# Wangshihu12/colmap-pcd

Hardware: AMD Instinct MI355X
Metric: NN queries/sec + BA-iter ms, 10M-pt cloud / 1M 3D feats (higher is better)
Workload: dtype f32 (NN distances) / f64 (association, BA); 1 GPU; M: 10000000-pt 'planes' cloud / 1000000 queries + BA scene 1000 cams / 1000000 pts / 4721253 obs / 900000 lidar terms (OPENCV), the same total at every N; cloud_points=10000000, queries=1000000, queries_this_rank=1000000, parallelism=single GPU

## Files before the change

### colmap-pcd_amd/csrc/ba.hip

```cpp
#include <algorithm>
#include <chrono>
#include <cmath>
#include <limits>
#include <memory>
#include <numeric>

#include "ba_cam_jac.h"
#include "ba_math.h"
#include "common.h"

namespace pcd {

struct BaDev {
  const int* cam_model; const int* cam_off; const double* cam_params;
  const double* poses; const int* image_cam; const uint8_t* image_const_pose; const uint8_t* image_const_tvec;
  const double* points; const uint8_t* point_const;
  const int* obs_image; const int* obs_point; const double* obs_xy;
  const int* lidar_point; const double* lidar_abcd; const double* lidar_w;
  const int* pt_order;
  const uint32_t* slice_start;
  const int* sell_img;
  const double* sell_xy;
  const uint32_t* pt_lidar_start; const uint32_t* pt_lidar_list;
  const uint32_t* img_obs_start;
  const int* img_pt;
  const uint32_t* img_obs;
  const uint32_t* seg_img;
  const uint32_t* seg_begin;
  const uint32_t* img_seg_start;
  const uint8_t* cam_refine;
  const uint32_t* cam_img_start;
  const uint32_t* cam_img_list;
  int C;
  int cam_k;
  const double* img_xy;
  int I, P, nslices; uint64_t O, L;
  int loss_type; double loss_scale;
};

template <int MODEL>
__device__ __forceinline__ void eval_block(const BaDev& d, int im, const double X[3], double ox, double oy,
                                           ReprojBlock& b, double q[4]) {
  const double* pose = d.poses + 7 * (size_t)im;
  double t[3];
#pragma unroll
  for (int k = 0; k < 4; ++k) q[k] = pose[k];
#pragma unroll
  for (int k = 0; k < 3; ++k) t[k] = pose[4 + k];
  const int cm = d.image_cam[im];
  const int model = MODEL >= 0 ? MODEL : d.cam_model[cm];
  reproj_eval(model, d.cam_params + d.cam_off[cm], q, t, X, ox, oy, b);
}

template <int N>
__device__ __forceinline__ void wave_store_rows(double* __restrict__ out, uint64_t row0, int cnt, const double (&v)[N],
                                                double* __restrict__ lds) {
  static_assert(N % 2 == 0, "rows are moved in 16-byte units");
  const int lane = threadIdx.x & 63;
#pragma unroll
  for (int k = 0; k < N; ++k) lds[lane * N + k] = v[k];
  __builtin_amdgcn_fence(__ATOMIC_RELEASE, "workgroup");
  __builtin_amdgcn_wave_barrier();
  __builtin_amdgcn_fence(__ATOMIC_ACQUIRE, "workgroup");
  const double2* src = reinterpret_cast<const double2*>(lds);
  double2* dst = reinterpret_cast<double2*>(out + row0 * N);
  const int units = cnt * (N / 2);
#pragma unroll
  for (int j = 0; j < N / 2; ++j) {
    const int u = j * 64 + lane;
    if (u < units) dst[u] = src[u];
  }
  __builtin_amdgcn_fence(__ATOMIC_RELEASE, "workgroup");
  __builtin_amdgcn_wave_barrier();
}

template <int MODEL, bool BLOCKS>
__global__ __launch_bounds__(256) void k_ba_points(BaDev d, double* __restrict__ Hpt, double* __restrict__ gpt,
                                                   double* __restrict__ cost_partial) {
  __shared__ double s_half[2][64][9];
  const int sl = threadIdx.x >> 7, half = (threadIdx.x >> 6) & 1, lane = threadIdx.x & 63;
  const int slice = blockIdx.x * 2 + sl;
  const int t = slice * 64 + lane;
  double cost = 0.0;
  double H[6] = {0, 0, 0, 0, 0, 0}, g[3] = {0, 0, 0};
  int p = -1;
  bool cpt = true;
  double X[3] = {0, 0, 0};
  if (slice < d.nslices) {
    p = d.pt_order[t];
    const uint32_t s0 = d.slice_start[slice], s1 = d.slice_start[slice + 1];
    if (p >= 0) {
      X[0] = d.points[3 * (size_t)p]; X[1] = d.points[3 * (size_t)p + 1]; X[2] = d.points[3 * (size_t)p + 2];
      cpt = d.point_const && d.point_const[p];
    }
    for (uint32_t s = s0 + lane + 64u * half; s < s1; s += 128) {
      const int im = d.sell_img[s];
      if (im < 0) continue;
      ReprojBlock b;
      double q[4];
      eval_block<MODEL>(d, im, X, d.sell_xy[2 * (size_t)s], d.sell_xy[2 * (size_t)s + 1], b, q);
      double rho0, rho1;
      loss_eval(d.loss_type, d.loss_scale, b.r[0] * b.r[0] + b.r[1] * b.r[1], rho0, rho1);
      cost += 0.5 * rho0;
      if (BLOCKS && !cpt) {
        const double sr = sqrt(rho1);
        double J[6];
#pragma unroll
        for (int r = 0; r < 2; ++r)
#pragma unroll
          for (int k = 0; k < 3; ++k)
            J[3 * r + k] = sr * (b.M[3 * r] * b.D[k] + b.M[3 * r + 1] * b.D[3 + k] + b.M[3 * r + 2] * b.D[6 + k]);
        const double r0 = sr * b.r[0], r1 = sr * b.r[1];
        H[0] += J[0] * J[0] + J[3] * J[3]; H[1] += J[0] * J[1] + J[3] * J[4]; H[2] += J[0] * J[2] + J[3] * J[5];
        H[3] += J[1] * J[1] + J[4] * J[4]; H[4] += J[1] * J[2] + J[4] * J[5]; H[5] += J[2] * J[2] + J[5] * J[5];
        g[0] += J[0] * r0 + J[3] * r1; g[1] += J[1] * r0 + J[4] * r1; g[2] += J[2] * r0 + J[5] * r1;
      }
    }
  }
  if (BLOCKS && half == 1) {
#pragma unroll
    for (int k = 0; k < 6; ++k) s_half[sl][lane][k] = H[k];
#pragma unroll
    for (int k = 0; k < 3; ++k) s_half[sl][lane][6 + k] = g[k];
  }
  __syncthreads();
  if (half == 0 && slice < d.nslices) {
    if (BLOCKS) {
#pragma unroll
      for (int k = 0; k < 6; ++k) H[k] += s_half[sl][lane][k];
#pragma unroll
      for (int k = 0; k < 3; ++k) g[k] += s_half[sl][lane][6 + k];
    }
    if (p >= 0) {
      for (uint32_t e = d.pt_lidar_start[p]; e < d.pt_lidar_start[p + 1]; ++e) {
        const uint32_t l = d.pt_lidar_list[e];
        const double abcd[4] = {d.lidar_abcd[4 * (size_t)l], d.lidar_abcd[4 * (size_t)l + 1],
                                d.lidar_abcd[4 * (size_t)l + 2], d.lidar_abcd[4 * (size_t)l + 3]};
        double r, J[3];
        lidar_eval(X, abcd, d.lidar_w[l], 0, r, J);
        double rho0, rho1;
        loss_eval(d.loss_type, d.loss_scale, r * r, rho0, rho1);
        cost += 0.5 * rho0;
        if (BLOCKS && !cpt) {
          const double sr = sqrt(rho1);
          const double rc = sr * r;
          J[0] *= sr; J[1] *= sr; J[2] *= sr;
          H[0] += J[0] * J[0]; H[1] += J[0] * J[1]; H[2] += J[0] * J[2];
          H[3] += J[1] * J[1]; H[4] += J[1] * J[2]; H[5] += J[2] * J[2];
          g[0] += J[0] * rc; g[1] += J[1] * rc; g[2] += J[2] * rc;
        }
      }
      if (BLOCKS && Hpt) {
        double* h = Hpt + 9 * (size_t)p;
        h[0] = H[0]; h[1] = H[1]; h[2] = H[2]; h[3] = H[1]; h[4] = H[3]; h[5] = H[4]; h[6] = H[2]; h[7] = H[4]; h[8] = H[5];
      }
      if (BLOCKS && gpt) { gpt[3 * (size_t)p] = g[0]; gpt[3 * (size_t)p + 1] = g[1]; gpt[3 * (size_t)p + 2] = g[2]; }
    }
  }
  __syncthreads();
  __shared__ double s_c[256];
  s_c[threadIdx.x] = cost;
  __syncthreads();
  for (int off = 128; off > 0; off >>= 1) {
    if ((int)threadIdx.x < off) s_c[threadIdx.x] += s_c[threadIdx.x + off];
    __syncthreads();
  }
  if (threadIdx.x == 0) cost_partial[blockIdx.x] = s_c[0];
}

template <int MODEL>
__global__ __launch_bounds__(256) void k_ba_cost(BaDev d, double* __restrict__ cost_partial) {
  double cost = 0.0;
  for (uint64_t i = blockIdx.x * (uint64_t)256 + threadIdx.x; i < d.O + d.L; i += (uint64_t)gridDim.x * 256) {
    if (i < d.O) {
      const int im = d.obs_image[i], pt = d.obs_point[i];
      const double X[3] = {d.points[3 * (size_t)pt], d.points[3 * (size_t)pt + 1], d.points[3 * (size_t)pt + 2]};
      ReprojBlock b;
      double q[4];
      eval_block<MODEL>(d, im, X, d.obs_xy[2 * i], d.obs_xy[2 * i + 1], b, q);
      double rho0, rho1;
      loss_eval(d.loss_type, d.loss_scale, b.r[0] * b.r[0] + b.r[1] * b.r[1], rho0, rho1);
      cost += 0.5 * rho0;
    } else {
      const uint64_t l = i - d.O;
      const int pt = d.lidar_point[l];
      const double X[3] = {d.points[3 * (size_t)pt], d.points[3 * (size_t)pt + 1], d.points[3 * (size_t)pt + 2]};
      const double abcd[4] = {d.lidar_abcd[4 * l], d.lidar_abcd[4 * l + 1], d.lidar_abcd[4 * l + 2], d.lidar_abcd[4 * l + 3]};
      double r, J[3];
      lidar_eval(X, abcd, d.lidar_w[l], 0, r, J);
      double rho0, rho1;
      loss_eval(d.loss_type, d.loss_scale, r * r, rho0, rho1);
      cost += 0.5 * rho0;
    }
  }
  __shared__ double s_c[256];
  s_c[threadIdx.x] = cost;
  __syncthreads();
  for (int off = 128; off > 0; off >>= 1) {
    if ((int)threadIdx.x < off) s_c[threadIdx.x] += s_c[threadIdx.x + off];
    __syncthreads();
  }
  if (threadIdx.x == 0) cost_partial[blockIdx.x] = s_c[0];
}
constexpr unsigned kCostBlocks = 1u << 20;

__global__ __launch_bounds__(256) void k_sum_partials(const double* __restrict__ partial, int n, double* __restrict__ out) {
  __shared__ double s_c[256];
  double a0 = 0.0, a1 = 0.0, a2 = 0.0, a3 = 0.0;
  int i = threadIdx.x;
  for (; i + 768 < n; i += 1024) { a0 += partial[i]; a1 += partial[i + 256]; a2 += partial[i + 512]; a3 += partial[i + 768]; }
  for (; i < n; i += 256) a0 += partial[i];
  s_c[threadIdx.x] = (a0 + a1) + (a2 + a3);
  __syncthreads();
  for (int off = 128; off > 0; off >>= 1) {
    if ((int)threadIdx.x < off) s_c[threadIdx.x] += s_c[threadIdx.x + off];
    __syncthreads();
  }
  if (threadIdx.x == 0) out[0] = s_c[0];
}

constexpr uint32_t kImgSeg = 1024;
template <int MODEL, bool WANT_W>
__global__ __launch_bounds__(256) void k_ba_images(BaDev d, double* __restrict__ partial, double* __restrict__ W_o) {
  __shared__ __attribute__((aligned(16))) double s_w[WANT_W ? 4 : 1][WANT_W ? 64 * 18 : 2];
  const int im = (int)d.seg_img[blockIdx.x];
  const int lane = threadIdx.x & 63;
  const int wave = __builtin_amdgcn_readfirstlane((int)(threadIdx.x >> 6));
  const bool cpose = d.image_const_pose && d.image_const_pose[im];
  double acc[27];
#pragma unroll
  for (int k = 0; k < 27; ++k) acc[k] = 0.0;
  const unsigned tmask = d.image_const_tvec ? d.image_const_tvec[im] : 0u;
  const uint32_t e_beg = d.seg_begin[blockIdx.x];
  const uint32_t e_end = min(d.seg_begin[blockIdx.x + 1], d.img_obs_start[im + 1]);
  if (!cpose || WANT_W) {
    for (uint32_t e0 = e_beg; e0 < e_end; e0 += 256) {
      const uint32_t e = e0 + threadIdx.x;
      const bool active = e < e_end;
      double w[18];
#pragma unroll
      for (int k = 0; k < 18; ++k) w[k] = 0.0;
      if (active && !cpose) {
        const int pt = d.img_pt[e];
        const double X[3] = {d.points[3 * (size_t)pt], d.points[3 * (size_t)pt + 1], d.points[3 * (size_t)pt + 2]};
        ReprojBlock b;
        double q[4];
        eval_block<MODEL>(d, im, X, d.img_xy[2 * (size_t)e], d.img_xy[2 * (size_t)e + 1], b, q);
        double rho0, rho1;
        loss_eval(d.loss_type, d.loss_scale, b.r[0] * b.r[0] + b.r[1] * b.r[1], rho0, rho1);
        const double sr = sqrt(rho1);
        double Jq[8], Jt[6], JX[6], Jqt[6];
        reproj_jacobians(b, Jq, Jt, JX);
        quat_tangent(q, Jq, Jqt);
        double J[12];
#pragma unroll
        for (int r = 0; r < 2; ++r)
#pragma unroll
          for (int k = 0; k < 3; ++k) {
            J[6 * r + k] = sr * Jqt[3 * r + k];
            J[6 * r + 3 + k] = ((tmask >> k) & 1u) ? 0.0 : sr * Jt[3 * r + k];
          }
        const double r0 = sr * b.r[0], r1 = sr * b.r[1];
        int idx = 0;
#pragma unroll
        for (int a = 0; a < 6; ++a)
#pragma unroll
          for (int c = a; c < 6; ++c) acc[idx++] += J[a] * J[c] + J[6 + a] * J[6 + c];
#pragma unroll
        for (int a = 0; a < 6; ++a) acc[21 + a] += J[a] * r0 + J[6 + a] * r1;
        if (WANT_W && !(d.point_const && d.point_const[pt])) {
#pragma unroll
          for (int a = 0; a < 6; ++a)
#pragma unroll
            for (int c = 0; c < 3; ++c) w[3 * a + c] = J[a] * (sr * JX[c]) + J[6 + a] * (sr * JX[3 + c]);
        }
      }
      if (WANT_W) {
        const uint32_t o = active ? d.img_obs[e] : 0u;
        const uint32_t o_first = (uint32_t)__builtin_amdgcn_readfirstlane((int)o);
        const int cnt = (int)min(64u, e_end > e0 + wave * 64u ? e_end - (e0 + wave * 64u) : 0u);
        const bool contiguous = __all(!active || o == o_first + (uint32_t)lane);
        if (contiguous) {
          wave_store_rows<18>(W_o, o_first, cnt, w, s_w[wave]);
        } else if (active) {
          double* dst = W_o + 18 * (size_t)o;
#pragma unroll
          for (int k = 0; k < 18; ++k) dst[k] = w[k];
        }
      }
    }
  }
  __shared__ double s_a[4][27];
#pragma unroll
  for (int k = 0; k < 27; ++k) {
    double v = acc[k];
#pragma unroll
    for (int off = 32; off > 0; off >>= 1) v += __shfl_xor(v, off);
    if (lane == 0) s_a[wave][k] = v;
  }
  __syncthreads();
  if (threadIdx.x < 27)
    partial[27 * (size_t)blockIdx.x + threadIdx.x] =
        (s_a[0][threadIdx.x] + s_a[1][threadIdx.x]) + (s_a[2][threadIdx.x] + s_a[3][threadIdx.x]);
}

__global__ __launch_bounds__(64) void k_ba_images_reduce(BaDev d, const double* __restrict__ partial,
                                                         double* __restrict__ Himg, double* __restrict__ gimg) {
  const int im = blockIdx.x * 2 + (threadIdx.x >> 5), k = threadIdx.x & 31;
  if (im >= d.I || k >= 27) return;
  double v = 0.0;
  for (uint32_t sgm = d.img_seg_start[im]; sgm < d.img_seg_start[im + 1]; ++sgm) v += partial[27 * (size_t)sgm + k];
  if (k >= 21) {
    if (gimg) gimg[6 * (size_t)im + (k - 21)] = v;
  } else if (Himg) {
    int a = 0, kk = k;
    while (kk >= 6 - a) { kk -= 6 - a; ++a; }
    const int c = a + kk;
    Himg[36 * (size_t)im + 6 * a + c] = v;
    Himg[36 * (size_t)im + 6 * c + a] = v;
  }
}

__host__ __device__ constexpr int cam_ne(int K) { return K * (K + 1) / 2 + 6 * K + K; }
__host__ __device__ constexpr int cam_ent_l(int K, int e) {
  const int ncc = K * (K + 1) / 2;
  if (e < ncc) { int a = 0; while (e >= K - a) { e -= K - a; ++a; } return a; }
  e -= ncc;
  if (e < 6 * K) return e / 6;
  return e - 6 * K;
}
__host__ __device__ constexpr int cam_ent_r(int K, int e) {
  const int ncc = K * (K + 1) / 2;
  if (e < ncc) { int a = 0; while (e >= K - a) { e -= K - a; ++a; } return a + e; }
  e -= ncc;
  if (e < 6 * K) return K + e % 6;
  return K + 6;
}

template <int MODEL, int CH>
__device__ __forceinline__ void cam_accumulate(const BaDev& d, int im, double* __restrict__ partial) {
  constexpr int K = MODEL >= 0 ? cam_num_params(MODEL >= 0 ? MODEL : 0) : PCD_CAM_JAC_STRIDE;
  constexpr int NE = cam_ne(K), PER = (NE + 3) / 4, E0 = CH * PER, E1 = E0 + PER < NE ? E0 + PER : NE;
  constexpr int NA = K + 7;
  const int lane = threadIdx.x & 63;
  const bool cpose = d.image_const_pose && d.image_const_pose[im];
  const unsigned tmask = d.image_const_tvec ? d.image_const_tvec[im] : 0u;
  const int cm = d.image_cam[im];
  const double* cam = d.cam_params + d.cam_off[cm];
  const uint8_t* refine = d.cam_refine ? d.cam_refine + d.cam_off[cm] : nullptr;
  const int model = MODEL >= 0 ? MODEL : d.cam_model[cm];
  double acc[PER > 0 ? PER : 1];
#pragma unroll
  for (int t = 0; t < PER; ++t) acc[t] = 0.0;
  for (uint32_t e = d.img_obs_start[im] + lane; e < d.img_obs_start[im + 1]; e += 64) {
    const int pt = d.img_pt[e];
    const double X[3] = {d.points[3 * (size_t)pt], d.points[3 * (size_t)pt + 1], d.points[3 * (size_t)pt + 2]};
    ReprojBlock b;
    double q[4];
    eval_block<MODEL>(d, im, X, d.img_xy[2 * (size_t)e], d.img_xy[2 * (size_t)e + 1], b, q);
    double rho0, rho1;
    loss_eval(d.loss_type, d.loss_scale, b.r[0] * b.r[0] + b.r[1] * b.r[1], rho0, rho1);
    const double sr = sqrt(rho1);
    double A[2][NA];
    {
      const double* pose = d.poses + 7 * (size_t)im;
      const double w = pose[0], a = pose[1], bq = pose[2], c = pose[3];
      const double cx = bq * X[2] - c * X[1], cy = c * X[0] - a * X[2], cz = a * X[1] - bq * X[0];
      const double ux = 2.0 * cx, uy = 2.0 * cy, uz = 2.0 * cz;
      const double Px = X[0] + w * ux + (bq * uz - c * uy) + pose[4];
      const double Py = X[1] + w * uy + (c * ux - a * uz) + pose[5];
      const double Pz = X[2] + w * uz + (a * uy - bq * ux) + pose[6];
      const double iz = 1.0 / Pz;
      double Jc[2 * K];
#pragma unroll
      for (int k = 0; k < 2 * K; ++k) Jc[k] = 0.0;
      if (MODEL >= 0) cam_param_jacobian<(MODEL >= 0 ? MODEL : 0)>(cam, Px * iz, Py * iz, Jc, K);
      else cam_param_jacobian_any(model, cam, Px * iz, Py * iz, Jc, K);
      const int kn = MODEL >= 0 ? K : cam_num_params(model);
#pragma unroll
      for (int k = 0; k < K; ++k) {
        const bool var = refine && k < kn && refine[k < kn ? k : 0];
        A[0][k] = var ? sr * Jc[k] : 0.0;
        A[1][k] = var ? sr * Jc[K + k] : 0.0;
      }
    }
    double Jq[8], Jt[6], JX[6], Jqt[6];
    reproj_jacobians(b, Jq, Jt, JX);
    quat_tangent(q, Jq, Jqt);
#pragma unroll
    for (int r = 0; r < 2; ++r) {
#pragma unroll
      for (int k = 0; k < 3; ++k) {
        A[r][K + k] = cpose ? 0.0 : sr * Jqt[3 * r + k];
        A[r][K + 3 + k] = (cpose || ((tmask >> k) & 1u)) ? 0.0 : sr * Jt[3 * r + k];
      }
      A[r][K + 6] = sr * b.r[r];
    }
#pragma unroll
    for (int t = 0; t < PER; ++t) {
      if (E0 + t < E1) {
        const int l = cam_ent_l(K, E0 + t), r = cam_ent_r(K, E0 + t);
        acc[t] += A[0][l] * A[0][r] + A[1][l] * A[1][r];
      }
    }
  }
#pragma unroll
  for (int t = 0; t < PER; ++t) {
    if (E0 + t < E1) {
      double v = acc[t];
#pragma unroll
      for (int off = 32; off > 0; off >>= 1) v += __shfl_xor(v, off);
      if (lane == 0) partial[(size_t)im * cam_ne(PCD_CAM_JAC_STRIDE) + E0 + t] = v;
    }
  }
}

template <int MODEL>
__global__ __launch_bounds__(256) void k_ba_cameras(BaDev d, double* __restrict__ partial) {
  const int im = blockIdx.x;
  switch (threadIdx.x >> 6) {
    case 0: cam_accumulate<MODEL, 0>(d, im, partial); break;
    case 1: cam_accumulate<MODEL, 1>(d, im, partial); break;
    case 2: cam_accumulate<MODEL, 2>(d, im, partial); break;
    default: cam_accumulate<MODEL, 3>(d, im, partial); break;
  }
}

__global__ __launch_bounds__(256) void k_ba_cameras_reduce(BaDev d, const double* __restrict__ partial,
                                                           double* __restrict__ Hcam, double* __restrict__ gcam,
                                                           double* __restrict__ Ecam) {
  constexpr int S = PCD_CAM_JAC_STRIDE, NEMAX = cam_ne(S);
  const int c = blockIdx.x;
  const int model = d.cam_model[c];
  const int K = d.cam_k;
  (void)model;
  const int ncc = K * (K + 1) / 2, NE = ncc + 7 * K;
  for (int e = threadIdx.x; e < S * S + S; e += 256) {
    if (e < S * S) { if (Hcam) Hcam[(size_t)c * S * S + e] = 0.0; }
    else if (gcam) gcam[(size_t)c * S + (e - S * S)] = 0.0;
  }
  __syncthreads();
  for (int e = threadIdx.x; e < NE; e += 256) {
    if (e >= ncc && e < ncc + 6 * K) continue;
    double v = 0.0;
    for (uint32_t j = d.cam_img_start[c]; j < d.cam_img_start[c + 1]; ++j)
      v += partial[(size_t)d.cam_img_list[j] * NEMAX + e];
    if (e < ncc) {
      int a = 0, k = e;
      while (k >= K - a) { k -= K - a; ++a; }
      const int b = a + k;
      if (Hcam) { Hcam[(size_t)c * S * S + a * S + b] = v; Hcam[(size_t)c * S * S + b * S + a] = v; }
    } else if (gcam) {
      gcam[(size_t)c * S + (e - ncc - 6 * K)] = v;
    }
  }
  if (Ecam) {
    for (uint32_t j = d.cam_img_start[c]; j < d.cam_img_start[c + 1]; ++j) {
      const uint32_t im = d.cam_img_list[j];
      for (int e = threadIdx.x; e < S * 6; e += 256) {
        const int a = e / 6;
        Ecam[(size_t)im * S * 6 + e] = a < K ? partial[(size_t)im * NEMAX + ncc + e] : 0.0;
      }
    }
  }
}

template <int MODEL>
__global__ __launch_bounds__(256) void k_ba_cam_w(BaDev d, double* __restrict__ Wc_o) {
  constexpr int S = PCD_CAM_JAC_STRIDE;
  __shared__ __attribute__((aligned(16))) double s_rows[4][64 * 3 * S];
  const int wave = threadIdx.x >> 6;
  const uint64_t o = blockIdx.x * (uint64_t)256 + threadIdx.x;
  const uint64_t o_wave = blockIdx.x * (uint64_t)256 + wave * 64;
  if (o_wave >= d.O) return;
  const int cnt = (int)min((uint64_t)64, d.O - o_wave);
  double Wc[3 * S];
#pragma unroll
  for (int k = 0; k < 3 * S; ++k) Wc[k] = 0.0;
  if (o < d.O) {
    const int im = d.obs_image[o], pt = d.obs_point[o];
    const bool cpt = d.point_const && d.point_const[pt];
    const int cm = d.image_cam[im];
    const uint8_t* refine = d.cam_refine ? d.cam_refine + d.cam_off[cm] : nullptr;
    if (!cpt && refine) {
      const double X[3] = {d.points[3 * (size_t)pt], d.points[3 * (size_t)pt + 1], d.points[3 * (size_t)pt + 2]};
      ReprojBlock b;
      double q[4];
      eval_block<MODEL>(d, im, X, d.obs_xy[2 * o], d.obs_xy[2 * o + 1], b, q);
      double rho0, rho1;
      loss_eval(d.loss_type, d.loss_scale, b.r[0] * b.r[0] + b.r[1] * b.r[1], rho0, rho1);
      double Jq[8], Jt[6], JX[6];
      reproj_jacobians(b, Jq, Jt, JX);
      const double* pose = d.poses + 7 * (size_t)im;
      const double w = pose[0], a = pose[1], bq = pose[2], c = pose[3];
      const double cx = bq * X[2] - c * X[1], cy = c * X[0] - a * X[2], cz = a * X[1] - bq * X[0];
      const double ux = 2.0 * cx, uy = 2.0 * cy, uz = 2.0 * cz;
      const double Px = X[0] + w * ux + (bq * uz - c * uy) + pose[4];
      const double Py = X[1] + w * uy + (c * ux - a * uz) + pose[5];
      const double Pz = X[2] + w * uz + (a * uy - bq * ux) + pose[6];
      const double iz = 1.0 / Pz;
      const int model = MODEL >= 0 ? MODEL : d.cam_model[cm];
      double Jc[2 * S];
#pragma unroll
      for (int k = 0; k < 2 * S; ++k) Jc[k] = 0.0;
      if (MODEL >= 0) cam_param_jacobian<(MODEL >= 0 ? MODEL : 0)>(d.cam_params + d.cam_off[cm], Px * iz, Py * iz, Jc, S);
      else cam_param_jacobian_any(model, d.cam_params + d.cam_off[cm], Px * iz, Py * iz, Jc, S);
      const int kn = cam_num_params(model);
#pragma unroll
      for (int k = 0; k < S; ++k) {
        const bool var = k < kn && refine[k < kn ? k : 0];
#pragma unroll
        for (int j = 0; j < 3; ++j)
          Wc[3 * k + j] = var ? rho1 * (Jc[k] * JX[j] + Jc[S + k] * JX[3 + j]) : 0.0;
      }
    }
  }
  wave_store_rows<3 * S>(Wc_o, o_wave, cnt, Wc, s_rows[wave]);
}

template <int MODEL>
__global__ __launch_bounds__(256) void k_ba_raw(BaDev d, double* __restrict__ residuals, double* __restrict__ Jq_o,
                                                double* __restrict__ Jt_o, double* __restrict__ JX_o,
                                                double* __restrict__ W_o) {
  __shared__ __attribute__((aligned(16))) double s_rows[4][64 * 18];
  const int wave = threadIdx.x >> 6;
  const uint64_t o = blockIdx.x * (uint64_t)256 + threadIdx.x;
  const uint64_t o_wave = blockIdx.x * (uint64_t)256 + wave * 64;
  if (o_wave >= d.O) return;
  const int cnt = (int)min((uint64_t)64, d.O - o_wave);
  const bool active = o < d.O;
  double res[2] = {0, 0}, Jq[8], Jt[6], JX[6], Wb[18];
#pragma unroll
  for (int k = 0; k < 8; ++k) Jq[k] = 0.0;
#pragma unroll
  for (int k = 0; k < 6; ++k) { Jt[k] = 0.0; JX[k] = 0.0; }
#pragma unroll
  for (int k = 0; k < 18; ++k) Wb[k] = 0.0;
  if (active) {
    const int im = d.obs_image[o], pt = d.obs_point[o];
    const double X[3] = {d.points[3 * (size_t)pt], d.points[3 * (size_t)pt + 1], d.points[3 * (size_t)pt + 2]};
    ReprojBlock b;
    double q[4];
    eval_block<MODEL>(d, im, X, d.obs_xy[2 * o], d.obs_xy[2 * o + 1], b, q);
    reproj_jacobians(b, Jq, Jt, JX);
    const bool cpose = d.image_const_pose && d.image_const_pose[im];
    res[0] = b.r[0]; res[1] = b.r[1];
    if (W_o) {
      double rho0, rho1;
      loss_eval(d.loss_type, d.loss_scale, b.r[0] * b.r[0] + b.r[1] * b.r[1], rho0, rho1);
      const double sr = sqrt(rho1);
      const unsigned tmask = d.image_const_tvec ? d.image_const_tvec[im] : 0u;
      const bool cpt = d.point_const && d.point_const[pt];
      double Jqt[6], J[12], Jx[6];
      quat_tangent(q, Jq, Jqt);
#pragma unroll
      for (int r = 0; r < 2; ++r)
#pragma unroll
        for (int k = 0; k < 3; ++k) {
          J[6 * r + k] = cpose ? 0.0 : sr * Jqt[3 * r + k];
          J[6 * r + 3 + k] = (cpose || ((tmask >> k) & 1u)) ? 0.0 : sr * Jt[3 * r + k];
          Jx[3 * r + k] = cpt ? 0.0 : sr * JX[3 * r + k];
        }
#pragma unroll
      for (int a = 0; a < 6; ++a)
#pragma unroll
        for (int c = 0; c < 3; ++c) Wb[3 * a + c] = J[a] * Jx[c] + J[6 + a] * Jx[3 + c];
    }
    if (cpose) {
#pragma unroll
      for (int k = 0; k < 8; ++k) Jq[k] = 0.0;
#pragma unroll
      for (int k = 0; k < 6; ++k) Jt[k] = 0.0;
    }
  }
  if (residuals) wave_store_rows<2>(residuals, o_wave, cnt, res, s_rows[wave]);
  if (Jq_o) wave_store_rows<8>(Jq_o, o_wave, cnt, Jq, s_rows[wave]);
  if (Jt_o) wave_store_rows<6>(Jt_o, o_wave, cnt, Jt, s_rows[wave]);
  if (JX_o) wave_store_rows<6>(JX_o, o_wave, cnt, JX, s_rows[wave]);
  if (W_o) wave_store_rows<18>(W_o, o_wave, cnt, Wb, s_rows[wave]);
}

template <int MODEL>
__global__ __launch_bounds__(256) void k_ba_cam_jac(BaDev d, double* __restrict__ Jc_o) {
  const uint64_t o = blockIdx.x * (uint64_t)256 + threadIdx.x;
  if (o >= d.O) return;
  const int im = d.obs_image[o], pt = d.obs_point[o];
  const double* pose = d.poses + 7 * (size_t)im;
  const double* Xp = d.points + 3 * (size_t)pt;
  const double X[3] = {Xp[0], Xp[1], Xp[2]};
  const double w = pose[0], a = pose[1], bq = pose[2], c = pose[3];
  const double cx = bq * X[2] - c * X[1], cy = c * X[0] - a * X[2], cz = a * X[1] - bq * X[0];
  const double ux = 2.0 * cx, uy = 2.0 * cy, uz = 2.0 * cz;
  const double Px = X[0] + w * ux + (bq * uz - c * uy) + pose[4];
  const double Py = X[1] + w * uy + (c * ux - a * uz) + pose[5];
  const double Pz = X[2] + w * uz + (a * uy - bq * ux) + pose[6];
  const double iz = 1.0 / Pz;
  const int cm = d.image_cam[im];
  double J[2 * PCD_CAM_JAC_STRIDE];
#pragma unroll
  for (int k = 0; k < 2 * PCD_CAM_JAC_STRIDE; ++k) J[k] = 0.0;
  if (MODEL >= 0) cam_param_jacobian<(MODEL >= 0 ? MODEL : 0)>(d.cam_params + d.cam_off[cm], Px * iz, Py * iz, J, PCD_CAM_JAC_STRIDE);
  else cam_param_jacobian_any(d.cam_model[cm], d.cam_params + d.cam_off[cm], Px * iz, Py * iz, J, PCD_CAM_JAC_STRIDE);
  double* out = Jc_o + 2 * PCD_CAM_JAC_STRIDE * o;
#pragma unroll
  for (int k = 0; k < 2 * PCD_CAM_JAC_STRIDE; ++k) out[k] = J[k];
}
// ... 1866 lines not shown
```

Baseline: 740.7 million queries/s.

## Accumulate per-image camera Hessian and gradient with f64 MFMA via LDS-staged rows

Replaces the per-thread 27-register accumulation of J^T J and J^T r for camera blocks with a 16x16x4 f64 MFMA outer-product accumulate. Each wave stages its Jacobian rows and weighted residuals in the shared W transpose scratch, then feeds them to the matrix core. This removes the per-lane FMA work and the 27 shuffle reductions at the end. In exchange it adds LDS round-trips and wave barriers per 256-observation chunk, enlarges shared memory for all instantiations, and changes launch bounds (min 4 blocks per SM for model 4 with W), which may alter register allocation and floating-point summation order.

```diff
diff --git a/colmap-pcd_amd/csrc/ba.hip b/colmap-pcd_amd/csrc/ba.hip
--- a/colmap-pcd_amd/csrc/ba.hip
+++ b/colmap-pcd_amd/csrc/ba.hip
@@ -220,26 +220,36 @@
 }
 
 constexpr uint32_t kImgSeg = 1024;
+constexpr int kRowColStride = 132;
+static_assert(7 * kRowColStride <= 64 * 18, "the staged rows share the W transpose scratch");
+typedef double mfma_f64x4 __attribute__((ext_vector_type(4)));
+
 template <int MODEL, bool WANT_W>
-__global__ __launch_bounds__(256) void k_ba_images(BaDev d, double* __restrict__ partial, double* __restrict__ W_o) {
-  __shared__ __attribute__((aligned(16))) double s_w[WANT_W ? 4 : 1][WANT_W ? 64 * 18 : 2];
+__global__ __launch_bounds__(256, (MODEL == 4 && WANT_W) ? 4 : 1) void k_ba_images(BaDev d, double* __restrict__ partial,
+                                                                       double* __restrict__ W_o) {
+  __shared__ __attribute__((aligned(16))) double s_w[4][64 * 18];
+  __shared__ double s_a[4][2][27];
   const int im = (int)d.seg_img[blockIdx.x];
   const int lane = threadIdx.x & 63;
   const int wave = __builtin_amdgcn_readfirstlane((int)(threadIdx.x >> 6));
   const bool cpose = d.image_const_pose && d.image_const_pose[im];
-  double acc[27];
-#pragma unroll
-  for (int k = 0; k < 27; ++k) acc[k] = 0.0;
+  mfma_f64x4 acc = {0.0, 0.0, 0.0, 0.0};
   const unsigned tmask = d.image_const_tvec ? d.image_const_tvec[im] : 0u;
   const uint32_t e_beg = d.seg_begin[blockIdx.x];
   const uint32_t e_end = min(d.seg_begin[blockIdx.x + 1], d.img_obs_start[im + 1]);
+  const int op_k = lane >> 4, op_c = (lane & 7) == 7 ? 0 : (lane & 7);
+  const double* op_src = s_w[wave] + op_c * kRowColStride + 2 * op_k + ((lane >> 3) & 1);
   if (!cpose || WANT_W) {
     for (uint32_t e0 = e_beg; e0 < e_end; e0 += 256) {
       const uint32_t e = e0 + threadIdx.x;
       const bool active = e < e_end;
+      const int cnt = (int)min(64u, e_end > e0 + wave * 64u ? e_end - (e0 + wave * 64u) : 0u);
       double w[18];
 #pragma unroll
       for (int k = 0; k < 18; ++k) w[k] = 0.0;
+      double J[12], r0 = 0.0, r1 = 0.0;
+#pragma unroll
+      for (int k = 0; k < 12; ++k) J[k] = 0.0;
       if (active && !cpose) {
         const int pt = d.img_pt[e];
         const double X[3] = {d.points[3 * (size_t)pt], d.points[3 * (size_t)pt + 1], d.points[3 * (size_t)pt + 2]};
@@ -252,7 +262,6 @@
         double Jq[8], Jt[6], JX[6], Jqt[6];
         reproj_jacobians(b, Jq, Jt, JX);
         quat_tangent(q, Jq, Jqt);
-        double J[12];
 #pragma unroll
         for (int r = 0; r < 2; ++r)
 #pragma unroll
@@ -260,25 +269,34 @@
             J[6 * r + k] = sr * Jqt[3 * r + k];
             J[6 * r + 3 + k] = ((tmask >> k) & 1u) ? 0.0 : sr * Jt[3 * r + k];
           }
-        const double r0 = sr * b.r[0], r1 = sr * b.r[1];
-        int idx = 0;
-#pragma unroll
-        for (int a = 0; a < 6; ++a)
-#pragma unroll
-          for (int c = a; c < 6; ++c) acc[idx++] += J[a] * J[c] + J[6 + a] * J[6 + c];
-#pragma unroll
-        for (int a = 0; a < 6; ++a) acc[21 + a] += J[a] * r0 + J[6 + a] * r1;
+        r0 = sr * b.r[0];
+        r1 = sr * b.r[1];
         if (WANT_W && !(d.point_const && d.point_const[pt])) {
 #pragma unroll
           for (int a = 0; a < 6; ++a)
 #pragma unroll
             for (int c = 0; c < 3; ++c) w[3 * a + c] = J[a] * (sr * JX[c]) + J[6 + a] * (sr * JX[3 + c]);
         }
+      }
+      if (!cpose && cnt > 0) {
+        double2* row_dst = reinterpret_cast<double2*>(s_w[wave]) + lane;
+#pragma unroll
+        for (int c = 0; c < 6; ++c) row_dst[c * (kRowColStride / 2)] = make_double2(J[c], J[6 + c]);
+        row_dst[6 * (kRowColStride / 2)] = make_double2(r0, r1);
+        __builtin_amdgcn_fence(__ATOMIC_RELEASE, "workgroup");
+        __builtin_amdgcn_wave_barrier();
+        __builtin_amdgcn_fence(__ATOMIC_ACQUIRE, "workgroup");
+#pragma unroll
+        for (int s = 0; s < 16; ++s) {
+          const double a = op_src[8 * s];
+          acc = __builtin_amdgcn_mfma_f64_16x16x4f64(a, a, acc, 0, 0, 0);
+        }
+        __builtin_amdgcn_fence(__ATOMIC_RELEASE, "workgroup");
+        __builtin_amdgcn_wave_barrier();
       }
       if (WANT_W) {
         const uint32_t o = active ? d.img_obs[e] : 0u;
         const uint32_t o_first = (uint32_t)__builtin_amdgcn_readfirstlane((int)o);
-        const int cnt = (int)min(64u, e_end > e0 + wave * 64u ? e_end - (e0 + wave * 64u) : 0u);
         const bool contiguous = __all(!active || o == o_first + (uint32_t)lane);
         if (contiguous) {
           wave_store_rows<18>(W_o, o_first, cnt, w, s_w[wave]);
@@ -290,18 +308,21 @@
       }
     }
   }
-  __shared__ double s_a[4][27];
-#pragma unroll
-  for (int k = 0; k < 27; ++k) {
-    double v = acc[k];
-#pragma unroll
-    for (int off = 32; off > 0; off >>= 1) v += __shfl_xor(v, off);
-    if (lane == 0) s_a[wave][k] = v;
+  {
+    const int g = lane >> 4, h = (lane >> 3) & 1, c = lane & 7;
+#pragma unroll
+    for (int hi = 0; hi < 2; ++hi) {
+      const int a = g + 4 * hi;
+      const double v = h ? acc[2 + hi] : acc[hi];
+      if (a < 6 && c >= a && c < 7) s_a[wave][h][c == 6 ? 21 + a : a * 6 - a * (a - 1) / 2 + (c - a)] = v;
+    }
   }
   __syncthreads();
-  if (threadIdx.x < 27)
-    partial[27 * (size_t)blockIdx.x + threadIdx.x] =
-        (s_a[0][threadIdx.x] + s_a[1][threadIdx.x]) + (s_a[2][threadIdx.x] + s_a[3][threadIdx.x]);
+  if (threadIdx.x < 27) {
+    const int k = threadIdx.x;
+    partial[27 * (size_t)blockIdx.x + k] = ((s_a[0][0][k] + s_a[0][1][k]) + (s_a[1][0][k] + s_a[1][1][k])) +
+                                           ((s_a[2][0][k] + s_a[2][1][k]) + (s_a[3][0][k] + s_a[3][1][k]));
+  }
 }
 
 __global__ __launch_bounds__(64) void k_ba_images_reduce(BaDev d, const double* __restrict__ partial,
```

Measured after the change: 753.2 million queries/s, median of 6. 1.7% higher.
